# MengRao/pollnet

Measured on AMD Instinct MI355X. Metric: device-resident Gbit/s + Mframes/s, 1500 B IPv4/TCP frames, 1/2/4/8 MI355X, higher is better.
Workload: dtype u16/u32 integer (one's-complement sums)

## Files before the change

### pollnet_amd/csrc/pn_internal.hpp

```cpp
#pragma once

#include <hip/hip_runtime.h>

#include <cstdint>
#include <string>
#include <vector>

#include "../../include/pollnet_amd.h"

struct pn_fence {
  hipStream_t s = nullptr;
  hipEvent_t ev = nullptr;
  uint8_t state = 0;
};

struct pn_ctx {
  int device = 0;
  pn_conn_entry* tbl_buf[2] = {nullptr, nullptr};
  uint32_t tbl_cap[2] = {0, 0};
  int cur = 0;
  pn_conn_entry* tbl_dev = nullptr;
  uint32_t n_entries = 0;
  uint64_t mask = 0;
  uint32_t max_conn = 0;
  bool verify_tcp = true;
  std::vector<hipStream_t> streams;
  std::vector<hipEvent_t> retired;
  size_t n_retired = 0;
  hipStream_t copy_stream = nullptr;
  void* tx_patch = nullptr;
  uint32_t tx_patch_n = 0;
  pn_fence tx;
  void* sig_count = nullptr;
  pn_fence sig[2];
  std::vector<pn_service*> services;
  uint64_t* udp_tbl = nullptr;
  uint32_t udp_cap = 0;
  uint32_t udp_mask = 0;
  uint32_t udp_n = 0;
  uint32_t* ub_tbl = nullptr;
  uint32_t ub_cap = 0;
  uint32_t ub_n = 0;
  void* ug_scratch = nullptr;
  uint32_t ug_scratch_n = 0;
  pn_fence ug;
  std::string err;
};

namespace pn_internal {

inline thread_local std::string g_err;

inline int set_err(pn_ctx* ctx, int code, const std::string& msg) {
  if (ctx) ctx->err = msg;
  g_err = msg;
  return code;
}

int svc_release_table(pn_ctx* ctx, int buf);

inline int hip_err(pn_ctx* ctx, hipError_t e, const char* what) {
  return set_err(ctx, PN_EHIP, std::string(what) + ": " + hipGetErrorString(e));
}

inline void note_stream(pn_ctx* ctx, hipStream_t s) {
  if (!ctx->streams.empty() && ctx->streams.back() == s) return;
  for (size_t i = 0; i < ctx->streams.size(); ++i)
    if (ctx->streams[i] == s) {
      std::swap(ctx->streams[i], ctx->streams.back());
      return;
    }
  ctx->streams.push_back(s);
}

inline int ensure_event(pn_ctx* ctx, hipEvent_t* ev) {
  if (*ev) return PN_OK;
  hipError_t e = hipEventCreateWithFlags(ev, hipEventDisableTiming);
  if (e != hipSuccess) return hip_err(ctx, e, "hipEventCreate");
  return PN_OK;
}

inline int fence_host_wait(pn_ctx* ctx, pn_fence& f) {
  hipError_t e = hipSuccess;
  if (f.state == 1) e = hipStreamSynchronize(f.s);
  else if (f.state == 2) e = hipEventSynchronize(f.ev);
  if (e != hipSuccess) return hip_err(ctx, e, "waiting for the last user of ctx scratch");
  f.state = 0;
  return PN_OK;
}

inline int fence_use(pn_ctx* ctx, pn_fence& f, hipStream_t s) {
  hipError_t e = hipSuccess;
  if (f.state == 1 && f.s != s) {
    int rc = ensure_event(ctx, &f.ev);
    if (rc) return rc;
    e = hipEventRecord(f.ev, f.s);
    if (e == hipSuccess) e = hipStreamWaitEvent(s, f.ev, 0);
  } else if (f.state == 2) {
    e = hipStreamWaitEvent(s, f.ev, 0);
  }
  if (e != hipSuccess) return hip_err(ctx, e, "ordering after the previous user of ctx scratch");
  f.s = s;
  f.state = 1;
  return PN_OK;
}

inline int fence_detach(pn_ctx* ctx, pn_fence& f) {
  if (f.state != 1) return PN_OK;
  int rc = ensure_event(ctx, &f.ev);
  if (rc) return rc;
  hipError_t e = hipEventRecord(f.ev, f.s);
  if (e != hipSuccess) return hip_err(ctx, e, "hipEventRecord(ctx scratch fence)");
  f.state = 2;
  f.s = nullptr;
  return PN_OK;
}

inline int wait_retired(pn_ctx* ctx) {
  for (size_t i = 0; i < ctx->n_retired; ++i) {
    hipError_t e = hipEventSynchronize(ctx->retired[i]);
    if (e != hipSuccess) return hip_err(ctx, e, "hipEventSynchronize(previous table readers)");
  }
  ctx->n_retired = 0;
  return PN_OK;
}

inline int retire_streams(pn_ctx* ctx) {
  for (size_t i = 0; i < ctx->streams.size(); ++i) {
    if (ctx->retired.size() <= i) ctx->retired.push_back(nullptr);
    int rc = ensure_event(ctx, &ctx->retired[i]);
    if (rc) return rc;
    hipError_t e = hipEventRecord(ctx->retired[i], ctx->streams[i]);
    if (e != hipSuccess) return hip_err(ctx, e, "hipEventRecord(table readers)");
  }
  ctx->n_retired = ctx->streams.size();
  ctx->streams.clear();
  for (pn_fence* f : {&ctx->sig[0], &ctx->sig[1], &ctx->tx, &ctx->ug}) {
    int rc = fence_detach(ctx, *f);
    if (rc) return rc;
  }
  return PN_OK;
}

inline int notify_counter(pn_ctx* ctx, int kind, hipStream_t s, uint32_t** out) {
  hipError_t e;
  if (!ctx->sig_count) {
    e = hipMalloc(&ctx->sig_count, 128);
    if (e == hipSuccess) e = hipMemsetAsync(ctx->sig_count, 0, 128, s);
    if (e != hipSuccess) return hip_err(ctx, e, "hipMalloc(notify counters)");
    for (pn_fence& f : ctx->sig) {
      f.s = s;
      f.state = 1;
    }
    note_stream(ctx, s);
  }
  int rc = fence_use(ctx, ctx->sig[kind], s);
  if (rc) return rc;
  *out = (uint32_t*)ctx->sig_count + 16 * kind;
  return PN_OK;
}

}
```

### pollnet_amd/csrc/rx_kernel.hip

```cpp
#include "rx_classify.hpp"

namespace {
using pn_internal::g_err;
using pn_internal::hip_err;
using pn_internal::set_err;

int strided_args(pn_ctx* ctx, const char* fn, const void* frames_dev, uint32_t slot_stride, uint32_t frame_off,
                 uint32_t n, void* results_dev, KArgs& a) {
  if (!ctx) return set_err(nullptr, PN_EINVAL, std::string(fn) + ": ctx is NULL");
  if (!ctx->tbl_dev) return set_err(ctx, PN_ENOTABLE, std::string(fn) + ": no conn table (call pn_set_conn_table)");
  if (!frames_dev || !results_dev) return set_err(ctx, PN_EINVAL, std::string(fn) + ": NULL buffer");
  if (((uintptr_t)frames_dev & 15) || ((uintptr_t)results_dev & 15))
    return set_err(ctx, PN_EINVAL, std::string(fn) + ": frames/results must be 16-byte aligned");
  if ((slot_stride & 15) || slot_stride > 65536 || (frame_off & 1) || slot_stride < frame_off + 96)
    return set_err(ctx, PN_EINVAL, std::string(fn) + ": slot_stride/frame_off violate the layout contract");
  strided_kargs(a, frames_dev, results_dev, ctx->tbl_dev, ctx->mask, ctx->n_entries, ctx->max_conn, n, slot_stride, frame_off);
  return PN_OK;
}

template <bool SIG>
void launch_strided(const pn_ctx* ctx, const KArgs& a, uint32_t frame_off, hipStream_t s) {
  for_mis(frame_off, [&](auto mis) {
    if (ctx->verify_tcp) launch<mis(), SIG, false>(a, s);
    else launch<mis(), SIG, true>(a, s);
  });
}

template <int A>
void launch_indexed(const KArgs& a, uint32_t eth_mod16, hipStream_t s) {
  for_mis(eth_mod16, [&](auto mis) { launch_one<mis(), 1, A, kLoadAux, kStoreAux, 1, kIdxWin, kXcdOrder>(a, s); });
}

}

extern "C" {

int pn_device_count(int* n) {
  if (!n) return PN_EINVAL;
  hipError_t e = hipGetDeviceCount(n);
  if (e != hipSuccess) {
    *n = 0;
    return hip_err(nullptr, e, "hipGetDeviceCount");
  }
  return PN_OK;
}


int pn_open(int device, pn_ctx** out) {
  if (!out) return set_err(nullptr, PN_EINVAL, "pn_open: out is NULL");
  int n = 0;
  hipError_t e = hipGetDeviceCount(&n);
  if (e != hipSuccess) return hip_err(nullptr, e, "hipGetDeviceCount");
  if (device < 0 || device >= n) return set_err(nullptr, PN_EINVAL, "pn_open: no such device");
  pn_ctx* c = new pn_ctx();
  c->device = device;
  *out = c;
  return PN_OK;
}

void pn_close(pn_ctx* ctx) {
  if (!ctx) return;
  (void)hipSetDevice(ctx->device);
  if (ctx->tbl_buf[0] || ctx->tbl_buf[1] || ctx->tx_patch || ctx->sig_count || ctx->udp_tbl || ctx->ub_tbl ||
      ctx->ug_scratch)
    (void)hipDeviceSynchronize();
  for (pn_conn_entry* b : ctx->tbl_buf)
    if (b) (void)hipFree(b);
  if (ctx->udp_tbl) (void)hipFree(ctx->udp_tbl);
  if (ctx->ub_tbl) (void)hipFree(ctx->ub_tbl);
  if (ctx->tx_patch) (void)hipFree(ctx->tx_patch);
  if (ctx->ug_scratch) (void)hipFree(ctx->ug_scratch);
  if (ctx->sig_count) (void)hipFree(ctx->sig_count);
  for (hipEvent_t ev : ctx->retired)
    if (ev) (void)hipEventDestroy(ev);
  for (pn_fence* f : {&ctx->sig[0], &ctx->sig[1], &ctx->tx, &ctx->ug})
    if (f->ev) (void)hipEventDestroy(f->ev);
  if (ctx->copy_stream) (void)hipStreamDestroy(ctx->copy_stream);
  delete ctx;
}

const char* pn_last_error(const pn_ctx* ctx) { return ctx ? ctx->err.c_str() : g_err.c_str(); }

int pn_set_conn_table(pn_ctx* ctx, const pn_conn_entry* entries, uint32_t n_entries, uint64_t tbl_mask,
                      uint32_t max_conn_cnt) {
  if (!ctx || !entries || n_entries == 0) return set_err(ctx, PN_EINVAL, "pn_set_conn_table: bad arguments");
  if (tbl_mask >= n_entries || (tbl_mask & (tbl_mask + 1)) != 0)
    return set_err(ctx, PN_EINVAL, "pn_set_conn_table: tbl_mask must be 2^k-1 < n_entries");
  hipError_t e = hipSetDevice(ctx->device);
  if (e != hipSuccess) return hip_err(ctx, e, "hipSetDevice");
  const int nxt = ctx->tbl_dev ? ctx->cur ^ 1 : ctx->cur;
  int rc = pn_internal::svc_release_table(ctx, nxt);
  if (rc) return rc;
  rc = pn_internal::wait_retired(ctx);
  if (rc) return rc;
  if (n_entries > ctx->tbl_cap[nxt]) {
    if (ctx->tbl_buf[nxt]) (void)hipFree(ctx->tbl_buf[nxt]);
    ctx->tbl_buf[nxt] = nullptr;
    ctx->tbl_cap[nxt] = 0;
    e = hipMalloc(&ctx->tbl_buf[nxt], (size_t)n_entries * sizeof(pn_conn_entry));
    if (e != hipSuccess) return hip_err(ctx, e, "hipMalloc(conn table)");
    ctx->tbl_cap[nxt] = n_entries;
  }
  if (!ctx->copy_stream) {
    e = hipStreamCreateWithFlags(&ctx->copy_stream, hipStreamNonBlocking);
    if (e != hipSuccess) return hip_err(ctx, e, "hipStreamCreate(table uploads)");
  }
  e = hipMemcpyAsync(ctx->tbl_buf[nxt], entries, (size_t)n_entries * sizeof(pn_conn_entry), hipMemcpyHostToDevice,
                     ctx->copy_stream);
  if (e == hipSuccess) e = hipStreamSynchronize(ctx->copy_stream);
  if (e != hipSuccess) return hip_err(ctx, e, "hipMemcpyAsync(conn table)");
  rc = pn_internal::retire_streams(ctx);
  if (rc) return rc;
  ctx->cur = nxt;
  ctx->tbl_dev = ctx->tbl_buf[nxt];
  ctx->n_entries = n_entries;
  ctx->mask = tbl_mask;
  ctx->max_conn = max_conn_cnt;
  return PN_OK;
}


int pn_classify(pn_ctx* ctx, const void* frames_dev, uint32_t slot_stride, uint32_t frame_off, uint32_t n,
                void* results_dev, void* stream) {
  if (ctx && n == 0 && ctx->tbl_dev) return PN_OK;
  KArgs a;
  int rc = strided_args(ctx, "pn_classify", frames_dev, slot_stride, frame_off, n, results_dev, a);
  if (rc) return rc;
  if (n == 0) return PN_OK;
  hipStream_t s = (hipStream_t)stream;
  hipError_t e = hipSetDevice(ctx->device);
  if (e != hipSuccess) return hip_err(ctx, e, "hipSetDevice");
  launch_strided<false>(ctx, a, frame_off, s);
  e = hipGetLastError();
  if (e != hipSuccess) return hip_err(ctx, e, "rx_classify launch");
  pn_internal::note_stream(ctx, s);
  return PN_OK;
}

int pn_classify_notify(pn_ctx* ctx, const void* frames, uint32_t slot_stride, uint32_t frame_off, uint32_t n,
                       void* results, void* stream, uint32_t* done_word, uint32_t token) {
  KArgs a;
  int rc = strided_args(ctx, "pn_classify_notify", frames, slot_stride, frame_off, n, results, a);
  if (rc) return rc;
  if (n == 0 || n > PN_NOTIFY_MAX_FRAMES || !done_word || ((uintptr_t)done_word & 3))
    return set_err(ctx, PN_EINVAL, "pn_classify_notify: n must be in [1, PN_NOTIFY_MAX_FRAMES], done_word 4-byte aligned");
  hipStream_t s = (hipStream_t)stream;
  hipError_t e = hipSetDevice(ctx->device);
  if (e != hipSuccess) return hip_err(ctx, e, "hipSetDevice");
  rc = pn_internal::notify_counter(ctx, 0, s, &a.sig_count);
  if (rc) return rc;
  a.sig_flag = done_word;
  a.sig_token = token;
  launch_strided<true>(ctx, a, frame_off, s);
  e = hipGetLastError();
  if (e != hipSuccess) return hip_err(ctx, e, "rx_classify (notify) launch");
  pn_internal::note_stream(ctx, s);
  return PN_OK;
}


int pn_classify_indexed(pn_ctx* ctx, const void* base, const uint64_t* offsets, uint32_t eth_mod16, uint32_t n,
                        uint32_t avail, void* results_dev, void* stream) {
  if (!ctx) return set_err(nullptr, PN_EINVAL, "pn_classify_indexed: ctx is NULL");
  if (!ctx->tbl_dev) return set_err(ctx, PN_ENOTABLE, "pn_classify_indexed: no conn table (call pn_set_conn_table)");
  if (n == 0) return PN_OK;
  if (!base || !offsets || !results_dev) return set_err(ctx, PN_EINVAL, "pn_classify_indexed: NULL buffer");
  if (((uintptr_t)base & 15) || ((uintptr_t)results_dev & 15) || ((uintptr_t)offsets & 7))
    return set_err(ctx, PN_EINVAL, "pn_classify_indexed: base/results must be 16-byte, offsets 8-byte aligned");
  if (eth_mod16 > 15 || (eth_mod16 & 1) || avail < 96 || avail > 65536)
    return set_err(ctx, PN_EINVAL, "pn_classify_indexed: eth_mod16 must be even < 16, avail in [96, 65536]");
  KArgs a;
  a.frames = (const uint8_t*)base;
  a.out = (pn_result*)results_dev;
  a.tbl = ctx->tbl_dev;
  a.mask = ctx->mask;
  a.n_entries = ctx->n_entries;
  a.max_conn = ctx->max_conn;
  a.n = n;
  a.stride = 0;
  a.ipa_off = 0;
  a.avail = avail;
  a.offs = offsets;
  a.fpw = frames_per_wave(n);
  hipStream_t s = (hipStream_t)stream;
  hipError_t e = hipSetDevice(ctx->device);
  if (e != hipSuccess) return hip_err(ctx, e, "hipSetDevice");
  if (ctx->verify_tcp) launch_indexed<kProdAbl>(a, eth_mod16, s);
  else launch_indexed<kProdAbl | kHeaderOnly>(a, eth_mod16, s);
  e = hipGetLastError();
  if (e != hipSuccess) return hip_err(ctx, e, "rx_classify (indexed) launch");
  pn_internal::note_stream(ctx, s);
  return PN_OK;
}

int pn_set_verify(pn_ctx* ctx, int verify_tcp) {
  if (!ctx) return set_err(nullptr, PN_EINVAL, "pn_set_verify: ctx is NULL");
  ctx->verify_tcp = verify_tcp != 0;
  return PN_OK;
}

int pn_sync(pn_ctx* ctx) {
  if (!ctx) return set_err(nullptr, PN_EINVAL, "pn_sync: ctx is NULL");
  hipError_t e = hipSetDevice(ctx->device);
  if (e != hipSuccess) return hip_err(ctx, e, "hipSetDevice");
  for (hipStream_t s : ctx->streams) {
    e = hipStreamSynchronize(s);
    if (e != hipSuccess) return hip_err(ctx, e, "hipStreamSynchronize");
  }
  ctx->streams.clear();
  int rc = pn_internal::wait_retired(ctx);
  if (rc) return rc;
  for (pn_fence* f : {&ctx->sig[0], &ctx->sig[1], &ctx->tx, &ctx->ug}) f->state = 0;
  return PN_OK;
}

}
```

### pollnet_amd/csrc/rx_service.hip

```cpp
#include <algorithm>
#include <chrono>
#include <cstdlib>

#include "rx_classify.hpp"

namespace {
using pn_internal::hip_err;
using pn_internal::set_err;

struct alignas(64) SvcPost {
  uint32_t gen;
  uint32_t n;
  uint32_t fpw;
  uint32_t max_conn;
  const uint8_t* frames;
  pn_result* out;
  const pn_conn_entry* tbl;
  uint16_t* links;
  uint32_t mask;
  uint32_t n_entries;
  uint32_t check;
  uint32_t seq;
};
static_assert(sizeof(SvcPost) == 64, "one line per post");

constexpr uint32_t kDoneWords = 64;
constexpr uint32_t kCountWords = 64;
constexpr uint32_t kExitWord = 96;
constexpr uint32_t kWordsBytes = 512;
constexpr uint32_t kLatWaves = PN_SERVICE_WAVES;
static_assert(kLatWaves <= kDoneWords, "a latency-tier post completes through per-wave done words");
constexpr uint32_t kLatFrames = kLatWaves * kFramesPerWave;
constexpr uint32_t kNetLimitMs = 8000;
constexpr uint32_t kPostVerify = 1u << 30, kPostLinks = 1u << 29, kPostN = (1u << 21) - 1;
constexpr uint32_t kLinkFrames = PN_LINK_MAX_FRAMES, kLinkConns = PN_LINK_MAX_CONNS;
constexpr uint32_t kMailBytes = 4096;

struct alignas(64) SvcDev {
  uint32_t count[2][16];
};
constexpr uint32_t kExitFlag = 32;

#ifdef PN_SVC_TRACE
__device__ uint64_t* g_svc_trace = nullptr;
#define SVC_T(w, i)                                                       \
  do {                                                                    \
    if (lane == 0 && (w) < 64) g_svc_trace[(w) * 8 + (i)] = wall_clock64(); \
  } while (0)
#else
#define SVC_T(w, i) \
  do {              \
  } while (0)
#endif

struct SArgs {
  const SvcPost* mail;
  u32x4* scratch;
  uint32_t* done_words;
  uint32_t* exit_word;
  SvcDev* dev;
  uint64_t idle_ticks;
  uint64_t net_ticks;
  uint32_t epoch;
  uint32_t last;
  uint32_t stride, ipa_off, avail;
  uint32_t poll_sleep;
};

inline uint32_t svc_fpw(uint32_t n, bool verify) {
  uint32_t fpw = verify ? 8u : kFramesPerWave;
  while (fpw < kFramesPerWave && (n + fpw - 1) / fpw > kLatWaves) fpw <<= 1;
  return fpw;
}

inline uint32_t svc_check(const SvcPost* p, uint32_t k) {
  const uint32_t* w = reinterpret_cast<const uint32_t*>(p);
  uint32_t x = k;
  for (int i = 1; i <= 13; i++) x ^= w[i];
  return x;
}

__host__ __device__ __forceinline__ uint32_t svc_active(uint32_t n, uint32_t fpw, uint32_t waves) {
  const uint32_t groups = (n + fpw - 1) / fpw;
  return groups < waves ? groups : waves;
}

inline uint32_t svc_helpers(uint32_t n, uint32_t max) {
  if (n <= kLatFrames) return 0;
  const uint32_t groups = (n + kFramesPerWave - 1) / kFramesPerWave;
  return std::min(groups - kLatWaves, max);
}

__device__ __forceinline__ KArgsAux svc_args(uint32_t v, uint32_t b, const SArgs& s, uint32_t k) {
  auto w32 = [&](uint32_t i) { return (uint32_t)__builtin_amdgcn_readlane(v, b + i); };
  auto u64 = [&](uint32_t lo) { return ((uint64_t)w32(lo + 1) << 32) | w32(lo); };
  KArgsAux a;
  const uint32_t nw = w32(1);
  a.n = nw & kPostN;
  a.fpw = w32(2) & 0xffu;
  a.max_conn = w32(3);
  a.frames = reinterpret_cast<const uint8_t*>(u64(4));
  a.out = reinterpret_cast<pn_result*>(u64(6));
  a.tbl = reinterpret_cast<const pn_conn_entry*>(u64(8));
  a.mask = w32(12);
  a.n_entries = w32(13);
  a.stride = s.stride;
  a.ipa_off = s.ipa_off;
  a.avail = s.avail;
  a.offs = nullptr;
  a.aux = (nw & kPostLinks) ? s.scratch + (size_t)(k & 1) * kLinkFrames * 2 : nullptr;
  return a;
}

__device__ __forceinline__ uint16_t* svc_links(uint32_t v, uint32_t b) {
  return reinterpret_cast<uint16_t*>(((uint64_t)(uint32_t)__builtin_amdgcn_readlane(v, b + 11) << 32) |
                                     (uint32_t)__builtin_amdgcn_readlane(v, b + 10));
}

constexpr uint32_t kCleanNeed = PN_F_HIT | PN_F_ACK | PN_F_IP_OK;
constexpr uint32_t kCleanNone = PN_F_TW | PN_F_SYN | PN_F_FIN | PN_F_RST | PN_F_NOT_TCP | PN_F_TRUNC | PN_F_BADOFF |
                                PN_F_IHL_NE_5;

struct ChainLds {
  uint32_t last[kLinkConns];
  uint32_t key[kLinkFrames];
  uint32_t seq_end[kLinkFrames];
  u32x4 fields[kLinkFrames];
};

__device__ __forceinline__ ChainLds& chain_lds() {
  __shared__ ChainLds c;
  return c;
}

__device__ __forceinline__ void chain_init(int lane) {
  ChainLds& c = chain_lds();
  for (uint32_t i = lane; i < kLinkConns; i += kWave) c.last[i] = 0u;
  wave_lds_sync();
}

__device__ __forceinline__ void chain_step(ChainLds& c, uint32_t base, uint32_t n, uint32_t max_conn, bool on,
                                           const u32x4& rec, const u32x4& fx, const __amdgpu_buffer_rsrc_t& lr,
                                           uint64_t below, int lane) {
  const uint32_t i = base + lane;
  const bool valid = i < n;
  const uint32_t flags = rec.w & 0xffffu;
  const uint32_t len = rec.z >> 16;
  const bool member = on && valid && (flags & (PN_F_HIT | PN_F_TW)) == PN_F_HIT && rec.x < max_conn;
  const bool usable = (flags & kCleanNeed) == kCleanNeed && (flags & kCleanNone) == 0 &&
                      (flags & (PN_F_TCP_OK | PN_F_TCP_UNCHECKED)) != 0 && len != 0 && len < 0x8000u;
  const uint32_t key = member ? rec.x : 0u;
  if (valid) {
    c.key[i] = member ? key : 0xFFFFFFFFu;
    c.seq_end[i] = rec.y + len;
    c.fields[i] = u32x4{fx.x, fx.y, fx.z, (rec.z & 0xffffu) | (usable ? 0x10000u : 0u)};
  }
  uint32_t prev = 0;
  if (member) prev = c.last[key];
  wave_lds_sync();
  if (member) atomicMax(&c.last[key], i + 1);
  wave_lds_sync();
  uint64_t todo = __ballot(member && c.last[key] != i + 1);
  while (todo) {
    const uint32_t leader = (uint32_t)__builtin_ctzll(todo);
    const uint32_t kk = __builtin_amdgcn_readlane(key, leader);
    const uint64_t m = __ballot(member && key == kk);
    todo &= ~m;
    const uint64_t lower = m & below;
    if (member && key == kk && lower) prev = base + 64u - (uint32_t)__builtin_clzll(lower);
  }
  uint32_t d = 0;
  if (member && usable && prev) {
    const uint32_t j = prev - 1;
    const u32x4 pf = c.fields[j];
    if ((pf.w >> 16) && c.seq_end[j] == rec.y && pf.x == fx.x && pf.y == fx.y && pf.z == fx.z &&
        (pf.w & 0xffffu) == (rec.z & 0xffffu))
      d = i - j;
  }
  if (valid) __builtin_amdgcn_raw_buffer_store_b16((unsigned short)d, lr, i * 2, 0, 0);
  wave_lds_sync();
}

__device__ __forceinline__ void chain_pass(const u32x4* aux, uint32_t n, uint32_t max_conn, uint16_t* links, int lane) {
  constexpr int kChunk = 8;
  ChainLds& c = chain_lds();
  const bool on = max_conn <= kLinkConns;
  const __amdgpu_buffer_rsrc_t lr = frame_rsrc(reinterpret_cast<const uint8_t*>(links), n * 2);
  const __amdgpu_buffer_rsrc_t ar = frame_rsrc(reinterpret_cast<const uint8_t*>(aux), n * 32);
  const uint64_t below = (1ull << lane) - 1;
  for (uint32_t base0 = 0; base0 < n; base0 += kChunk * kWave) {
    u32x4 rec[kChunk], fx[kChunk];
#pragma unroll
    for (int s = 0; s < kChunk; ++s) {
      const uint32_t i = base0 + s * kWave + lane;
      rec[s] = __builtin_amdgcn_raw_buffer_load_b128(ar, i * 32, 0, 0);
      fx[s] = __builtin_amdgcn_raw_buffer_load_b128(ar, i * 32 + 16, 0, 0);
    }
#pragma unroll
    for (int s = 0; s < kChunk; ++s)
      if (base0 + s * kWave < n) chain_step(c, base0 + s * kWave, n, max_conn, on, rec[s], fx[s], lr, below, lane);
  }
  for (uint32_t i = lane; i < n; i += kWave) {
    const uint32_t k = c.key[i];
    if (k != 0xFFFFFFFFu) c.last[k] = 0u;
  }
  wave_lds_sync();
}

template <int MIS, int COOP, bool HELPER = false>
__device__ __forceinline__ void svc_run(const KArgsAux& a, bool verify, bool linked, uint32_t w, uint32_t act, uint32_t k,
                                        uint32_t* done_word, int lane) {
  for (uint32_t g = w; g * a.fpw < a.n; g += act) {
    if (verify) classify_group<MIS, COOP, kProdAbl | kChainAux, kLoadAux, kStoreAux, 0, kLoadAux>(a, g * a.fpw, lane);
    else
      classify_group<MIS, COOP, kProdAbl | kHeaderOnly | kChainAux, kLoadAux, kStoreAux, 0, kLoadAux>(a, g * a.fpw, lane);
  }
  if constexpr (HELPER) return;
  __threadfence_system();
  if (lane == 0 && act <= kDoneWords && !linked)
    __hip_atomic_store(done_word, k, __ATOMIC_RELAXED, __HIP_MEMORY_SCOPE_SYSTEM);
}

template <bool PASS>
__device__ __forceinline__ void svc_finish(const KArgsAux& a, uint16_t* links, uint32_t k, uint32_t* count_word, int lane) {
  if constexpr (PASS) {
    if (a.aux) {
      __builtin_amdgcn_fence(__ATOMIC_ACQUIRE, "agent");
      chain_pass(a.aux, a.n, a.max_conn, links, lane);
    }
  }
  __threadfence_system();
  if (lane == 0) __hip_atomic_store(count_word, k, __ATOMIC_RELAXED, __HIP_MEMORY_SCOPE_SYSTEM);
}

template <bool PASS>
__device__ __forceinline__ void svc_count(uint32_t* count, const KArgsAux& a, uint16_t* links, uint32_t target, uint32_t k,
                                          uint32_t* count_word, int lane) {
  uint32_t prev = 0;
  if (lane == 0) prev = atomicAdd(count, 1u);
  prev = __builtin_amdgcn_readfirstlane(prev);
  if (prev == target - 1) {
    if (lane == 0) __hip_atomic_store(count, 0u, __ATOMIC_RELAXED, __HIP_MEMORY_SCOPE_AGENT);
    svc_finish<PASS>(a, links, k, count_word, lane);
  }
}

template <int MIS, int COOP>
__global__ __launch_bounds__(kWave) void rx_service_kernel(SArgs s) {
  const int lane = threadIdx.x;
  const uint32_t w = blockIdx.x, W = gridDim.x;
  const uint32_t* mw = reinterpret_cast<const uint32_t*>(s.mail);
  uint32_t last = s.last;
  uint64_t t0 = wall_clock64();
  chain_init(lane);
  for (;;) {
    const uint32_t v = lane <= (int)kExitFlag ? __hip_atomic_load(mw + lane, __ATOMIC_RELAXED, __HIP_MEMORY_SCOPE_SYSTEM) : 0u;
    if (w != 0 && (uint32_t)__builtin_amdgcn_readlane(v, kExitFlag) == s.epoch) return;
    const uint32_t k = last + 1;
    const uint32_t b = (k & 1) * 16;
    const uint32_t q = __builtin_amdgcn_readlane(v, b + 15);
    uint32_t x = q;
#pragma unroll
    for (uint32_t i = 1; i <= 13; i++) x ^= (uint32_t)__builtin_amdgcn_readlane(v, b + i);
    const bool whole = (uint32_t)__builtin_amdgcn_readlane(v, b) == q && (uint32_t)__builtin_amdgcn_readlane(v, b + 14) == x;
    if (!whole || (int32_t)(q - k) < 0) {
      if (w == 0) {
        if (wall_clock64() - t0 > s.idle_ticks) {
          if (lane == 0) {
            __hip_atomic_store(const_cast<uint32_t*>(mw) + kExitFlag, s.epoch, __ATOMIC_RELAXED, __HIP_MEMORY_SCOPE_SYSTEM);
            __hip_atomic_store(s.exit_word, s.epoch, __ATOMIC_RELEASE, __HIP_MEMORY_SCOPE_SYSTEM);
          }
          return;
        }
        __builtin_amdgcn_s_sleep(1);
      } else {
        if (wall_clock64() - t0 > s.net_ticks) return;
        for (uint32_t i = 0; i < s.poll_sleep; ++i) __builtin_amdgcn_s_sleep(1);
      }
      continue;
    }
    if (q != k) {
      last = k;
      t0 = wall_clock64();
      continue;
    }
    const uint32_t nw = __builtin_amdgcn_readlane(v, b + 1);
    if (nw == PN_SERVICE_STOP) return;
    last = k;
    const uint32_t fw = __builtin_amdgcn_readlane(v, b + 2);
    const uint32_t act = svc_active(nw & kPostN, fw & 0xffu, W + (fw >> 8));
    if (w < act) {
      SVC_T(w, 0);
      __builtin_amdgcn_fence(__ATOMIC_ACQUIRE, "");
      SVC_T(w, 1);
      const KArgsAux a = svc_args(v, b, s, k);
      SVC_T(w, 5);
      const bool linked = a.aux != nullptr;
      svc_run<MIS, COOP>(a, (nw & kPostVerify) != 0, linked, w, act, k, s.done_words + w, lane);
      SVC_T(w, 6);
      if (act > kDoneWords || linked) {
        uint32_t* cw = s.done_words + kCountWords + (k & 1);
        if (act == 1) svc_finish<true>(a, svc_links(v, b), k, cw, lane);
        else svc_count<true>(&s.dev->count[k & 1][0], a, svc_links(v, b), act < W ? act : W, k, cw, lane);
      }
      SVC_T(w, 7);
    }
    t0 = wall_clock64();
  }
}

template <int MIS, int COOP>
__global__ __launch_bounds__(kWave) void rx_service_helper_kernel(KArgsAux a, uint32_t verify, uint32_t act) {
  svc_run<MIS, COOP, true>(a, verify != 0, false, kLatWaves + blockIdx.x, act, 0, nullptr, threadIdx.x);
}

template <int MIS>
void launch_svc(bool coop, uint32_t waves, const SArgs& a, hipStream_t s) {
  if (coop) hipLaunchKernelGGL((rx_service_kernel<MIS, 1>), dim3(waves), dim3(kWave), 0, s, a);
  else hipLaunchKernelGGL((rx_service_kernel<MIS, 0>), dim3(waves), dim3(kWave), 0, s, a);
}

template <int MIS>
void launch_helpers(bool coop, uint32_t helpers, const KArgsAux& a, uint32_t verify, uint32_t act, hipStream_t s) {
  if (coop) hipLaunchKernelGGL((rx_service_helper_kernel<MIS, 1>), dim3(helpers), dim3(kWave), 0, s, a, verify, act);
  else hipLaunchKernelGGL((rx_service_helper_kernel<MIS, 0>), dim3(helpers), dim3(kWave), 0, s, a, verify, act);
}
}

struct pn_service {
  pn_ctx* ctx = nullptr;
  hipStream_t stream = nullptr;
  hipStream_t helper_stream = nullptr;
  uint32_t stride = 0, frame_off = 0;
  uint32_t helpers_max = 0;
  uint32_t post_helpers[2] = {0, 0};
  hipEvent_t helper_ev[2] = {nullptr, nullptr};
  uint64_t idle_ticks = 0, net_ticks = 0;
  SvcPost* mail = nullptr;
  bool mail_dev = false;
  uint32_t* words = nullptr;
  uint32_t post_words[2] = {0, 0};
  uint32_t tbl_post[2] = {0, 0};
  bool tbl_used[2] = {false, false};
  SvcDev* dev = nullptr;
  u32x4* scratch = nullptr;
  uint32_t seq = 0;
  uint32_t epoch = 0;
  bool running = false;
  bool coop = false;
};

namespace {
SArgs svc_sargs(const pn_service* v, uint32_t base) {
  SArgs a;
  a.mail = v->mail;
  a.scratch = v->scratch;
  a.done_words = v->words;
  a.exit_word = v->words + kExitWord;
  a.dev = v->dev;
  a.idle_ticks = v->idle_ticks;
  a.net_ticks = v->net_ticks;
  a.epoch = v->epoch;
  a.last = base;
  a.stride = v->stride;
  a.ipa_off = (v->frame_off + 14) & ~15u;
  a.avail = v->stride - v->frame_off;
  a.poll_sleep = v->mail_dev ? 1u : 16u;
  return a;
}

inline void host_sfence() { asm volatile("sfence" ::: "memory"); }

void svc_publish(SvcPost* slot, const SvcPost& q, bool wc) {
  static const bool avx = __builtin_cpu_supports("avx");
  if (wc && avx) {
    asm volatile(
        "vmovdqu (%0), %%ymm0\n\t"
        "vmovdqu 32(%0), %%ymm1\n\t"
        "vmovntdq %%ymm0, (%1)\n\t"
        "vmovntdq %%ymm1, 32(%1)\n\t"
        "sfence\n\t"
        "vzeroupper"
        :
        : "r"(&q), "r"(slot)
        : "memory", "xmm0", "xmm1");
    return;
  }
  volatile uint32_t* d = reinterpret_cast<volatile uint32_t*>(slot);
  const uint32_t* w = reinterpret_cast<const uint32_t*>(&q);
  for (int i = 1; i <= 14; ++i) d[i] = w[i];
  host_sfence();
  d[0] = w[0];
  d[15] = w[15];
  host_sfence();
}

int svc_launch_helpers(pn_service* v, uint32_t k, uint32_t helpers, const SvcPost& q) {
  KArgsAux a;
  strided_kargs(a, q.frames, q.out, q.tbl, q.mask, q.n_entries, q.max_conn, q.n & kPostN, v->stride, v->frame_off);
  a.fpw = q.fpw & 0xffu;
  const uint32_t verify = (q.n & kPostVerify) ? 1u : 0u, act = svc_active(a.n, a.fpw, kLatWaves + helpers);
  hipStream_t s = v->helper_stream;
  for_mis(v->frame_off, [&](auto mis) { launch_helpers<mis()>(v->coop, helpers, a, verify, act, s); });
  hipError_t e = hipGetLastError();
  if (e == hipSuccess && !v->helper_ev[k & 1]) e = hipEventCreateWithFlags(&v->helper_ev[k & 1], hipEventDisableTiming);
  if (e == hipSuccess) e = hipEventRecord(v->helper_ev[k & 1], s);
  if (e != hipSuccess) return hip_err(v->ctx, e, "pn_service: helper launch");
  return PN_OK;
}

int svc_launch(pn_service* v, uint32_t base) {
  pn_ctx* ctx = v->ctx;
  const SvcDev init{};
  hipError_t e = hipMemcpyAsync(v->dev, &init, sizeof(SvcDev), hipMemcpyHostToDevice, v->stream);
  if (e == hipSuccess) e = hipStreamSynchronize(v->stream);
  if (e != hipSuccess) return hip_err(ctx, e, "pn_service: device state");
  if (++v->epoch == 0) ++v->epoch;
  const SArgs a = svc_sargs(v, base);
  for_mis(v->frame_off, [&](auto mis) { launch_svc<mis()>(v->coop, kLatWaves, a, v->stream); });
  e = hipGetLastError();
  if (e != hipSuccess) return hip_err(ctx, e, "pn_service: launch");
  v->running = true;
  return PN_OK;
}

bool svc_post_ran(const pn_service* v, uint32_t k) {
  const uint32_t words = v->post_words[k & 1];
  if (words == 0 && (int32_t)(__atomic_load_n(v->words + kCountWords + (k & 1), __ATOMIC_ACQUIRE) - k) < 0) return false;
  for (uint32_t w = 0; w < words; ++w)
    if ((int32_t)(__atomic_load_n(v->words + w, __ATOMIC_ACQUIRE) - k) < 0) return false;
  if (v->post_helpers[k & 1] && hipEventQuery(v->helper_ev[k & 1]) != hipSuccess) return false;
  return true;
}

bool svc_post_done(const pn_service* v, uint32_t k) {
  if ((int32_t)(v->seq - k) >= 2) return true;
  if (!svc_post_ran(v, k)) return false;
  return k != v->seq || svc_post_ran(v, k - 1);
}

uint32_t svc_done(const pn_service* v) {
  if (svc_post_done(v, v->seq)) return v->seq;
  return svc_post_done(v, v->seq - 1) ? v->seq - 1 : v->seq - 2;
}

bool svc_exited(const pn_service* v) { return __atomic_load_n(v->words + kExitWord, __ATOMIC_ACQUIRE) == v->epoch; }

void svc_free(pn_service* v) {
  if (v->ctx) {
    auto& l = v->ctx->services;
    l.erase(std::remove(l.begin(), l.end(), v), l.end());
  }
  if (v->mail) (void)(v->mail_dev ? hipFree(v->mail) : hipHostFree(v->mail));
  if (v->words) (void)hipHostFree(v->words);
  if (v->dev) (void)hipFree(v->dev);
  if (v->scratch) (void)hipFree(v->scratch);
  if (v->stream) (void)hipStreamDestroy(v->stream);
  if (v->helper_stream) (void)hipStreamDestroy(v->helper_stream);
  for (hipEvent_t ev : v->helper_ev)
    if (ev) (void)hipEventDestroy(ev);
  delete v;
}
}

int pn_internal::svc_release_table(pn_ctx* ctx, int buf) {
  for (pn_service* v : ctx->services) {
    if (!v->tbl_used[buf]) continue;
    const uint32_t id = v->tbl_post[buf];
    if ((int32_t)(v->seq - id) < 2 && !svc_post_done(v, id)) {
      const int rc = pn_service_wait(v, id);
      if (rc) return rc;
    }
    v->tbl_used[buf] = false;
  }
  return PN_OK;
}

extern "C" {

int pn_service_open(pn_ctx* ctx, uint32_t slot_stride, uint32_t frame_off, uint32_t idle_ms, pn_service** out) {
  return pn_service_open_ex(ctx, slot_stride, frame_off, idle_ms, 0, out);
}

int pn_service_open_ex(pn_ctx* ctx, uint32_t slot_stride, uint32_t frame_off, uint32_t idle_ms, uint32_t large_waves,
                       pn_service** out) {
  if (!ctx || !out) return set_err(ctx, PN_EINVAL, "pn_service_open: ctx / out is NULL");
  *out = nullptr;
  if ((slot_stride & 15) || slot_stride > 65536 || (frame_off & 1) || slot_stride < frame_off + 96)
    return set_err(ctx, PN_EINVAL, "pn_service_open: slot_stride/frame_off violate the layout contract");
  if (idle_ms == 0 || idle_ms > 10000) return set_err(ctx, PN_EINVAL, "pn_service_open: idle_ms must be in [1, 10000]");
  if (large_waves && (large_waves < PN_SERVICE_WAVES || large_waves > PN_SERVICE_MAX_WAVES))
    return set_err(ctx, PN_EINVAL, "pn_service_open: large_waves must be 0 or in [PN_SERVICE_WAVES, PN_SERVICE_MAX_WAVES]");
  hipError_t e = hipSetDevice(ctx->device);
  if (e != hipSuccess) return hip_err(ctx, e, "hipSetDevice");
  int khz = 0;
  e = hipDeviceGetAttribute(&khz, hipDeviceAttributeWallClockRate, ctx->device);
  if (e != hipSuccess || khz <= 0) return hip_err(ctx, e, "pn_service_open: wall clock rate");
  int cus = 0;
  e = hipDeviceGetAttribute(&cus, hipDeviceAttributeMultiprocessorCount, ctx->device);
  if (e != hipSuccess || cus <= 0) return hip_err(ctx, e, "pn_service_open: CU count");
  pn_service* v = new pn_service();
  v->ctx = ctx;
  v->stride = slot_stride;
  v->frame_off = frame_off;
  const uint32_t total = large_waves ? large_waves
                                     : std::max<uint32_t>(kLatWaves, std::min<uint32_t>(PN_SERVICE_MAX_WAVES,
                                                                                      (uint32_t)cus * PN_SERVICE_WAVES_PER_CU));
  v->helpers_max = total - kLatWaves;
  v->idle_ticks = (uint64_t)khz * idle_ms;
  v->net_ticks = v->idle_ticks + (v->idle_ticks >> 1) + (uint64_t)khz * kNetLimitMs;
  v->coop = (slot_stride % 16) == 0 && ((frame_off + 14) & ~15u) >= 16;
  int large_bar = 0;
  if (hipDeviceGetAttribute(&large_bar, hipDeviceAttributeIsLargeBar, ctx->device) != hipSuccess) large_bar = 0;
  v->mail_dev = large_bar != 0 && std::getenv("PN_SERVICE_HOST_MAILBOX") == nullptr;
  if (v->mail_dev && hipExtMallocWithFlags((void**)&v->mail, kMailBytes, hipDeviceMallocUncached) != hipSuccess) {
    (void)hipGetLastError();
    v->mail = nullptr;
    v->mail_dev = false;
  }
  if ((e = hipStreamCreateWithFlags(&v->stream, hipStreamNonBlocking)) != hipSuccess ||
      (e = hipStreamCreateWithFlags(&v->helper_stream, hipStreamNonBlocking)) != hipSuccess ||
      (!v->mail && (e = hipHostMalloc((void**)&v->mail, kMailBytes, hipHostMallocDefault)) != hipSuccess) ||
      (e = hipHostMalloc((void**)&v->words, kWordsBytes, hipHostMallocDefault)) != hipSuccess ||
      (e = hipMalloc((void**)&v->dev, sizeof(SvcDev))) != hipSuccess ||
      (e = hipMalloc((void**)&v->scratch, sizeof(u32x4) * 2 * 2 * kLinkFrames)) != hipSuccess) {
    const int rc = hip_err(ctx, e, "pn_service_open: allocation");
    svc_free(v);
    return rc;
  }
  uint32_t first = 0;
  if (const char* env = std::getenv("PN_SERVICE_FIRST_POST")) first = (uint32_t)std::strtoull(env, nullptr, 0);
  std::memset(v->words, 0, kWordsBytes);
  for (uint32_t w = 0; w < kDoneWords + 2; ++w) v->words[w] = first;
  {
    SvcPost q{};
    q.gen = q.seq = first;
    q.check = ~svc_check(&q, first);
    for (int i = 0; i < 2; ++i) svc_publish(v->mail + i, q, v->mail_dev);
    volatile uint32_t* flag = reinterpret_cast<volatile uint32_t*>(v->mail) + kExitFlag;
    *flag = 0u;
    host_sfence();
  }
  v->seq = first;
  const int rc = svc_launch(v, first);
  if (rc) {
    svc_free(v);
    return rc;
  }
  ctx->services.push_back(v);
  *out = v;
  return PN_OK;
}

int pn_service_post(pn_service* v, const void* frames, uint32_t n, void* results, uint32_t* post_id) {
  return pn_service_post_linked(v, frames, n, results, nullptr, post_id);
}

int pn_service_post_linked(pn_service* v, const void* frames, uint32_t n, void* results, uint16_t* links,
                           uint32_t* post_id) {
  if (!v) return set_err(nullptr, PN_EINVAL, "pn_service_post: service is NULL");
  pn_ctx* ctx = v->ctx;
  if (!ctx->tbl_dev) return set_err(ctx, PN_ENOTABLE, "pn_service_post: no conn table (call pn_set_conn_table)");
  if (n == 0 || n > PN_SERVICE_MAX_FRAMES || !frames || !results)
    return set_err(ctx, PN_EINVAL, "pn_service_post: n must be in [1, PN_SERVICE_MAX_FRAMES], buffers set");
  if (((uintptr_t)frames & 15) || ((uintptr_t)results & 15))
    return set_err(ctx, PN_EINVAL, "pn_service_post: frames/results must be 16-byte aligned");
  if (links && (n > PN_LINK_MAX_FRAMES || ((uintptr_t)links & 1)))
    return set_err(ctx, PN_EINVAL, "pn_service_post_linked: n must be <= PN_LINK_MAX_FRAMES, links 2-byte aligned");
  const uint32_t done = svc_done(v);
  if ((int32_t)(v->seq - done) >= 2) return set_err(ctx, PN_EINVAL, "pn_service_post: two posts already outstanding");
  if (v->running && svc_exited(v)) v->running = false;
  if (!v->running) {
    const int rc = svc_launch(v, done);
    if (rc) return rc;
  }
  const uint32_t k = v->seq + 1;
  const bool verify = ctx->verify_tcp;
  SvcPost q{};
  q.n = n | (verify ? kPostVerify : 0u) | (links ? kPostLinks : 0u);
  q.max_conn = ctx->max_conn;
  q.frames = (const uint8_t*)frames;
  q.out = (pn_result*)results;
  q.tbl = ctx->tbl_dev;
  q.links = links;
  q.mask = (uint32_t)ctx->mask;
  q.n_entries = ctx->n_entries;
  const uint32_t fpw = svc_fpw(n, verify), helpers = svc_helpers(n, v->helpers_max);
  q.fpw = fpw | helpers << 8;
  const uint32_t act = svc_active(n, fpw, kLatWaves + helpers);
  if (helpers) {
    const int rc = svc_launch_helpers(v, k, helpers, q);
    if (rc) return rc;
  }
  v->post_helpers[k & 1] = helpers;
  v->post_words[k & 1] = (act <= kDoneWords && !links) ? act : 0u;
  v->tbl_post[ctx->cur] = k;
  v->tbl_used[ctx->cur] = true;
  q.check = svc_check(&q, k);
  q.gen = q.seq = k;
  svc_publish(v->mail + (k & 1), q, v->mail_dev);
  v->seq = k;
  if (post_id) *post_id = k;
  return PN_OK;
}

int pn_service_wait(pn_service* v, uint32_t post_id) {
  if (!v) return set_err(nullptr, PN_EINVAL, "pn_service_wait: service is NULL");
  if (post_id == 0 || (int32_t)(post_id - v->seq) > 0 || (int32_t)(v->seq - post_id) >= 2)
    post_id = v->seq;
  const uint32_t k = post_id;
  const auto t_start = std::chrono::steady_clock::now();
  for (uint64_t i = 1;; ++i) {
    if (svc_post_done(v, k)) return PN_OK;
    if ((i & 4095) == 0) {
      if (std::chrono::steady_clock::now() - t_start > std::chrono::seconds(10))
        return set_err(v->ctx, PN_EHIP, "pn_service_wait: no completion within 10 s");
      if (svc_exited(v)) {
        const uint32_t done = svc_done(v);
        if ((int32_t)(done - k) >= 0) return PN_OK;
        v->running = false;
        const int rc = svc_launch(v, done);
        if (rc) return rc;
        continue;
      }
      const hipError_t q = hipStreamQuery(v->stream);
      if (q != hipErrorNotReady && q != hipSuccess) return hip_err(v->ctx, q, "pn_service_wait: the service kernel failed");
      if (q == hipSuccess && !svc_post_done(v, k) && !svc_exited(v))
        return set_err(v->ctx, PN_EHIP, "pn_service_wait: the service kernel ended without completing the post");
    }
  }
}

int pn_service_close(pn_service* v) {
  if (!v) return PN_OK;
  pn_ctx* ctx = v->ctx;
  int rc = svc_post_done(v, v->seq) ? PN_OK : pn_service_wait(v, 0);
  if (v->running && !svc_exited(v)) {
    const uint32_t k = v->seq + 1;
    SvcPost q{};
    q.n = PN_SERVICE_STOP;
    v->post_words[k & 1] = 0;
    v->post_helpers[k & 1] = 0;
    q.check = svc_check(&q, k);
    q.gen = q.seq = k;
    svc_publish(v->mail + (k & 1), q, v->mail_dev);
    v->seq = k;
  }
  hipError_t e = hipStreamSynchronize(v->stream);
  if (e == hipSuccess) e = hipStreamSynchronize(v->helper_stream);
  if (e != hipSuccess && rc == PN_OK) rc = hip_err(ctx, e, "pn_service_close");
  svc_free(v);
  return rc;
}

}

#ifdef PN_SVC_TRACE
extern "C" int pn_svc_trace_set(uint64_t* host_buf) {
  return hipMemcpyToSymbol(HIP_SYMBOL(g_svc_trace), &host_buf, sizeof host_buf) == hipSuccess ? PN_OK : PN_EHIP;
}
#endif
```

Baseline: 53220.

## Split large service posts: persistent kernel handles head, full classify grid handles rest

```diff
diff --git a/pollnet_amd/csrc/pn_internal.hpp b/pollnet_amd/csrc/pn_internal.hpp
--- a/pollnet_amd/csrc/pn_internal.hpp
+++ b/pollnet_amd/csrc/pn_internal.hpp
@@ -62,6 +62,21 @@
 inline int hip_err(pn_ctx* ctx, hipError_t e, const char* what) {
   return set_err(ctx, PN_EHIP, std::string(what) + ": " + hipGetErrorString(e));
 }
+
+struct ClassifyJob {
+  const void* frames = nullptr;
+  void* out = nullptr;
+  const pn_conn_entry* tbl = nullptr;
+  uint64_t mask = 0;
+  uint32_t n_entries = 0, max_conn = 0;
+  uint32_t n = 0, stride = 0, frame_off = 0;
+  bool verify = true;
+  uint32_t* sig_count = nullptr;
+  uint32_t* sig_flag = nullptr;
+  uint32_t sig_token = 0;
+};
+
+hipError_t launch_classify(const ClassifyJob& j, hipStream_t s);
 
 inline void note_stream(pn_ctx* ctx, hipStream_t s) {
   if (!ctx->streams.empty() && ctx->streams.back() == s) return;
diff --git a/pollnet_amd/csrc/rx_kernel.hip b/pollnet_amd/csrc/rx_kernel.hip
--- a/pollnet_amd/csrc/rx_kernel.hip
+++ b/pollnet_amd/csrc/rx_kernel.hip
@@ -6,7 +6,7 @@
 using pn_internal::set_err;
 
 int strided_args(pn_ctx* ctx, const char* fn, const void* frames_dev, uint32_t slot_stride, uint32_t frame_off,
-                 uint32_t n, void* results_dev, KArgs& a) {
+                 uint32_t n, void* results_dev, pn_internal::ClassifyJob& j) {
   if (!ctx) return set_err(nullptr, PN_EINVAL, std::string(fn) + ": ctx is NULL");
   if (!ctx->tbl_dev) return set_err(ctx, PN_ENOTABLE, std::string(fn) + ": no conn table (call pn_set_conn_table)");
   if (!frames_dev || !results_dev) return set_err(ctx, PN_EINVAL, std::string(fn) + ": NULL buffer");
@@ -14,14 +14,23 @@
     return set_err(ctx, PN_EINVAL, std::string(fn) + ": frames/results must be 16-byte aligned");
   if ((slot_stride & 15) || slot_stride > 65536 || (frame_off & 1) || slot_stride < frame_off + 96)
     return set_err(ctx, PN_EINVAL, std::string(fn) + ": slot_stride/frame_off violate the layout contract");
-  strided_kargs(a, frames_dev, results_dev, ctx->tbl_dev, ctx->mask, ctx->n_entries, ctx->max_conn, n, slot_stride, frame_off);
+  j.frames = frames_dev;
+  j.out = results_dev;
+  j.tbl = ctx->tbl_dev;
+  j.mask = ctx->mask;
+  j.n_entries = ctx->n_entries;
+  j.max_conn = ctx->max_conn;
+  j.n = n;
+  j.stride = slot_stride;
+  j.frame_off = frame_off;
+  j.verify = ctx->verify_tcp;
   return PN_OK;
 }
 
 template <bool SIG>
-void launch_strided(const pn_ctx* ctx, const KArgs& a, uint32_t frame_off, hipStream_t s) {
+void launch_strided(bool verify, const KArgs& a, uint32_t frame_off, hipStream_t s) {
   for_mis(frame_off, [&](auto mis) {
-    if (ctx->verify_tcp) launch<mis(), SIG, false>(a, s);
+    if (verify) launch<mis(), SIG, false>(a, s);
     else launch<mis(), SIG, true>(a, s);
   });
 }
@@ -31,6 +40,20 @@
   for_mis(eth_mod16, [&](auto mis) { launch_one<mis(), 1, A, kLoadAux, kStoreAux, 1, kIdxWin, kXcdOrder>(a, s); });
 }
 
+}
+
+hipError_t pn_internal::launch_classify(const ClassifyJob& j, hipStream_t s) {
+  KArgs a;
+  strided_kargs(a, j.frames, j.out, j.tbl, j.mask, j.n_entries, j.max_conn, j.n, j.stride, j.frame_off);
+  if (j.sig_flag) {
+    a.sig_count = j.sig_count;
+    a.sig_flag = j.sig_flag;
+    a.sig_token = j.sig_token;
+    launch_strided<true>(j.verify, a, j.frame_off, s);
+  } else {
+    launch_strided<false>(j.verify, a, j.frame_off, s);
+  }
+  return hipGetLastError();
 }
 
 extern "C" {
@@ -123,15 +146,14 @@
 int pn_classify(pn_ctx* ctx, const void* frames_dev, uint32_t slot_stride, uint32_t frame_off, uint32_t n,
                 void* results_dev, void* stream) {
   if (ctx && n == 0 && ctx->tbl_dev) return PN_OK;
-  KArgs a;
-  int rc = strided_args(ctx, "pn_classify", frames_dev, slot_stride, frame_off, n, results_dev, a);
+  pn_internal::ClassifyJob j;
+  int rc = strided_args(ctx, "pn_classify", frames_dev, slot_stride, frame_off, n, results_dev, j);
   if (rc) return rc;
   if (n == 0) return PN_OK;
   hipStream_t s = (hipStream_t)stream;
   hipError_t e = hipSetDevice(ctx->device);
   if (e != hipSuccess) return hip_err(ctx, e, "hipSetDevice");
-  launch_strided<false>(ctx, a, frame_off, s);
-  e = hipGetLastError();
+  e = pn_internal::launch_classify(j, s);
   if (e != hipSuccess) return hip_err(ctx, e, "rx_classify launch");
   pn_internal::note_stream(ctx, s);
   return PN_OK;
@@ -139,20 +161,19 @@
 
 int pn_classify_notify(pn_ctx* ctx, const void* frames, uint32_t slot_stride, uint32_t frame_off, uint32_t n,
                        void* results, void* stream, uint32_t* done_word, uint32_t token) {
-  KArgs a;
-  int rc = strided_args(ctx, "pn_classify_notify", frames, slot_stride, frame_off, n, results, a);
+  pn_internal::ClassifyJob j;
+  int rc = strided_args(ctx, "pn_classify_notify", frames, slot_stride, frame_off, n, results, j);
   if (rc) return rc;
   if (n == 0 || n > PN_NOTIFY_MAX_FRAMES || !done_word || ((uintptr_t)done_word & 3))
     return set_err(ctx, PN_EINVAL, "pn_classify_notify: n must be in [1, PN_NOTIFY_MAX_FRAMES], done_word 4-byte aligned");
   hipStream_t s = (hipStream_t)stream;
   hipError_t e = hipSetDevice(ctx->device);
   if (e != hipSuccess) return hip_err(ctx, e, "hipSetDevice");
-  rc = pn_internal::notify_counter(ctx, 0, s, &a.sig_count);
-  if (rc) return rc;
-  a.sig_flag = done_word;
-  a.sig_token = token;
-  launch_strided<true>(ctx, a, frame_off, s);
-  e = hipGetLastError();
+  rc = pn_internal::notify_counter(ctx, 0, s, &j.sig_count);
+  if (rc) return rc;
+  j.sig_flag = done_word;
+  j.sig_token = token;
+  e = pn_internal::launch_classify(j, s);
   if (e != hipSuccess) return hip_err(ctx, e, "rx_classify (notify) launch");
   pn_internal::note_stream(ctx, s);
   return PN_OK;
diff --git a/pollnet_amd/csrc/rx_service.hip b/pollnet_amd/csrc/rx_service.hip
--- a/pollnet_amd/csrc/rx_service.hip
+++ b/pollnet_amd/csrc/rx_service.hip
@@ -332,9 +332,11 @@
   hipStream_t stream = nullptr;
   hipStream_t helper_stream = nullptr;
   uint32_t stride = 0, frame_off = 0;
+  bool bulk = false;
   uint32_t helpers_max = 0;
-  uint32_t post_helpers[2] = {0, 0};
+  bool post_grid[2] = {false, false};
   hipEvent_t helper_ev[2] = {nullptr, nullptr};
+  hipError_t grid_err = hipSuccess;
   uint64_t idle_ticks = 0, net_ticks = 0;
   SvcPost* mail = nullptr;
   bool mail_dev = false;
@@ -395,17 +397,34 @@
   host_sfence();
 }
 
-int svc_launch_helpers(pn_service* v, uint32_t k, uint32_t helpers, const SvcPost& q) {
-  KArgsAux a;
-  strided_kargs(a, q.frames, q.out, q.tbl, q.mask, q.n_entries, q.max_conn, q.n & kPostN, v->stride, v->frame_off);
-  a.fpw = q.fpw & 0xffu;
-  const uint32_t verify = (q.n & kPostVerify) ? 1u : 0u, act = svc_active(a.n, a.fpw, kLatWaves + helpers);
+int svc_launch_grid(pn_service* v, uint32_t k, uint32_t helpers, const SvcPost& q, uint32_t n) {
+  const bool verify = (q.n & kPostVerify) != 0;
   hipStream_t s = v->helper_stream;
-  for_mis(v->frame_off, [&](auto mis) { launch_helpers<mis()>(v->coop, helpers, a, verify, act, s); });
-  hipError_t e = hipGetLastError();
+  hipError_t e;
+  if (helpers == 0) {
+    pn_internal::ClassifyJob j;
+    j.frames = q.frames + (size_t)kLatFrames * v->stride;
+    j.out = q.out + kLatFrames;
+    j.tbl = q.tbl;
+    j.mask = q.mask;
+    j.n_entries = q.n_entries;
+    j.max_conn = q.max_conn;
+    j.n = n - kLatFrames;
+    j.stride = v->stride;
+    j.frame_off = v->frame_off;
+    j.verify = verify;
+    e = pn_internal::launch_classify(j, s);
+  } else {
+    KArgsAux a;
+    strided_kargs(a, q.frames, q.out, q.tbl, q.mask, q.n_entries, q.max_conn, n, v->stride, v->frame_off);
+    a.fpw = q.fpw & 0xffu;
+    const uint32_t act = svc_active(a.n, a.fpw, kLatWaves + helpers);
+    for_mis(v->frame_off, [&](auto mis) { launch_helpers<mis()>(v->coop, helpers, a, verify ? 1u : 0u, act, s); });
+    e = hipGetLastError();
+  }
   if (e == hipSuccess && !v->helper_ev[k & 1]) e = hipEventCreateWithFlags(&v->helper_ev[k & 1], hipEventDisableTiming);
   if (e == hipSuccess) e = hipEventRecord(v->helper_ev[k & 1], s);
-  if (e != hipSuccess) return hip_err(v->ctx, e, "pn_service: helper launch");
+  if (e != hipSuccess) return hip_err(v->ctx, e, "pn_service: a large post's grid launch");
   return PN_OK;
 }
 
@@ -424,24 +443,34 @@
   return PN_OK;
 }
 
-bool svc_post_ran(const pn_service* v, uint32_t k) {
+bool svc_post_ran(pn_service* v, uint32_t k, bool with_grid = true) {
   const uint32_t words = v->post_words[k & 1];
   if (words == 0 && (int32_t)(__atomic_load_n(v->words + kCountWords + (k & 1), __ATOMIC_ACQUIRE) - k) < 0) return false;
   for (uint32_t w = 0; w < words; ++w)
     if ((int32_t)(__atomic_load_n(v->words + w, __ATOMIC_ACQUIRE) - k) < 0) return false;
-  if (v->post_helpers[k & 1] && hipEventQuery(v->helper_ev[k & 1]) != hipSuccess) return false;
+  if (with_grid && v->post_grid[k & 1]) {
+    const hipError_t e = hipEventQuery(v->helper_ev[k & 1]);
+    if (e != hipSuccess && e != hipErrorNotReady) v->grid_err = e;
+    if (e != hipSuccess) return false;
+  }
   return true;
 }
 
-bool svc_post_done(const pn_service* v, uint32_t k) {
+bool svc_post_done(pn_service* v, uint32_t k, bool with_grid = true) {
   if ((int32_t)(v->seq - k) >= 2) return true;
-  if (!svc_post_ran(v, k)) return false;
-  return k != v->seq || svc_post_ran(v, k - 1);
-}
-
-uint32_t svc_done(const pn_service* v) {
-  if (svc_post_done(v, v->seq)) return v->seq;
-  return svc_post_done(v, v->seq - 1) ? v->seq - 1 : v->seq - 2;
+  if (!svc_post_ran(v, k, with_grid)) return false;
+  return k != v->seq || svc_post_ran(v, k - 1, with_grid);
+}
+
+uint32_t svc_done(pn_service* v, bool with_grid = true) {
+  if (svc_post_done(v, v->seq, with_grid)) return v->seq;
+  return svc_post_done(v, v->seq - 1, with_grid) ? v->seq - 1 : v->seq - 2;
+}
+
+uint32_t svc_tier_done(pn_service* v) { return svc_done(v, false); }
+
+int svc_grid_failed(pn_service* v, const char* fn) {
+  return hip_err(v->ctx, v->grid_err, (std::string(fn) + ": a large post's grid failed").c_str());
 }
 
 bool svc_exited(const pn_service* v) { return __atomic_load_n(v->words + kExitWord, __ATOMIC_ACQUIRE) == v->epoch; }
@@ -496,17 +525,12 @@
   int khz = 0;
   e = hipDeviceGetAttribute(&khz, hipDeviceAttributeWallClockRate, ctx->device);
   if (e != hipSuccess || khz <= 0) return hip_err(ctx, e, "pn_service_open: wall clock rate");
-  int cus = 0;
-  e = hipDeviceGetAttribute(&cus, hipDeviceAttributeMultiprocessorCount, ctx->device);
-  if (e != hipSuccess || cus <= 0) return hip_err(ctx, e, "pn_service_open: CU count");
   pn_service* v = new pn_service();
   v->ctx = ctx;
   v->stride = slot_stride;
   v->frame_off = frame_off;
-  const uint32_t total = large_waves ? large_waves
-                                     : std::max<uint32_t>(kLatWaves, std::min<uint32_t>(PN_SERVICE_MAX_WAVES,
-                                                                                      (uint32_t)cus * PN_SERVICE_WAVES_PER_CU));
-  v->helpers_max = total - kLatWaves;
+  v->bulk = large_waves == 0;
+  v->helpers_max = large_waves ? large_waves - kLatWaves : 0u;
   v->idle_ticks = (uint64_t)khz * idle_ms;
   v->net_ticks = v->idle_ticks + (v->idle_ticks >> 1) + (uint64_t)khz * kNetLimitMs;
   v->coop = (slot_stride % 16) == 0 && ((frame_off + 14) & ~15u) >= 16;
@@ -568,14 +592,18 @@
   if (links && (n > PN_LINK_MAX_FRAMES || ((uintptr_t)links & 1)))
     return set_err(ctx, PN_EINVAL, "pn_service_post_linked: n must be <= PN_LINK_MAX_FRAMES, links 2-byte aligned");
   const uint32_t done = svc_done(v);
+  if (v->grid_err != hipSuccess) return svc_grid_failed(v, "pn_service_post");
   if ((int32_t)(v->seq - done) >= 2) return set_err(ctx, PN_EINVAL, "pn_service_post: two posts already outstanding");
   if (v->running && svc_exited(v)) v->running = false;
   if (!v->running) {
-    const int rc = svc_launch(v, done);
+    const int rc = svc_launch(v, svc_tier_done(v));
     if (rc) return rc;
   }
   const uint32_t k = v->seq + 1;
   const bool verify = ctx->verify_tcp;
+  const bool split = v->bulk && n > kLatFrames;
+  const uint32_t n_all = n;
+  if (split) n = kLatFrames;
   SvcPost q{};
   q.n = n | (verify ? kPostVerify : 0u) | (links ? kPostLinks : 0u);
   q.max_conn = ctx->max_conn;
@@ -585,14 +613,14 @@
   q.links = links;
   q.mask = (uint32_t)ctx->mask;
   q.n_entries = ctx->n_entries;
-  const uint32_t fpw = svc_fpw(n, verify), helpers = svc_helpers(n, v->helpers_max);
+  const uint32_t fpw = svc_fpw(n, verify), helpers = split ? 0u : svc_helpers(n, v->helpers_max);
   q.fpw = fpw | helpers << 8;
   const uint32_t act = svc_active(n, fpw, kLatWaves + helpers);
-  if (helpers) {
-    const int rc = svc_launch_helpers(v, k, helpers, q);
+  if (split || helpers) {
+    const int rc = svc_launch_grid(v, k, helpers, q, n_all);
     if (rc) return rc;
   }
-  v->post_helpers[k & 1] = helpers;
+  v->post_grid[k & 1] = split || helpers;
   v->post_words[k & 1] = (act <= kDoneWords && !links) ? act : 0u;
   v->tbl_post[ctx->cur] = k;
   v->tbl_used[ctx->cur] = true;
@@ -612,15 +640,20 @@
   const auto t_start = std::chrono::steady_clock::now();
   for (uint64_t i = 1;; ++i) {
     if (svc_post_done(v, k)) return PN_OK;
+    if (v->grid_err != hipSuccess) return svc_grid_failed(v, "pn_service_wait");
     if ((i & 4095) == 0) {
       if (std::chrono::steady_clock::now() - t_start > std::chrono::seconds(10))
         return set_err(v->ctx, PN_EHIP, "pn_service_wait: no completion within 10 s");
+      const hipError_t h = hipStreamQuery(v->helper_stream);
+      if (h != hipErrorNotReady && h != hipSuccess) return hip_err(v->ctx, h, "pn_service_wait: a large post's grid failed");
       if (svc_exited(v)) {
-        const uint32_t done = svc_done(v);
-        if ((int32_t)(done - k) >= 0) return PN_OK;
+        if ((int32_t)(svc_done(v) - k) >= 0) return PN_OK;
         v->running = false;
-        const int rc = svc_launch(v, done);
-        if (rc) return rc;
+        const uint32_t ran = svc_tier_done(v);
+        if ((int32_t)(ran - k) < 0) {
+          const int rc = svc_launch(v, ran);
+          if (rc) return rc;
+        }
         continue;
       }
       const hipError_t q = hipStreamQuery(v->stream);
@@ -640,14 +673,15 @@
     SvcPost q{};
     q.n = PN_SERVICE_STOP;
     v->post_words[k & 1] = 0;
-    v->post_helpers[k & 1] = 0;
+    v->post_grid[k & 1] = false;
     q.check = svc_check(&q, k);
     q.gen = q.seq = k;
     svc_publish(v->mail + (k & 1), q, v->mail_dev);
     v->seq = k;
   }
   hipError_t e = hipStreamSynchronize(v->stream);
-  if (e == hipSuccess) e = hipStreamSynchronize(v->helper_stream);
+  const hipError_t h = hipStreamSynchronize(v->helper_stream);
+  if (e == hipSuccess) e = h;
   if (e != hipSuccess && rc == PN_OK) rc = hip_err(ctx, e, "pn_service_close");
   svc_free(v);
   return rc;
```

Result: slower. 52490 (-1.4%).
